# OrientalHorizon/Ray-Tracer-Archive

Measured on NVIDIA B200. Metric: path segments/sec, higher is better.
Workload: dtype f32

## Files before the change

ray_tracer_archive_b200/csrc/rtb_device.cuh:

```cuda
#pragma once
#include <cuda_runtime.h>
#include <stdint.h>

#include <cmath>
#include <cstring>

#include "rtb_internal.hpp"

namespace rtb {

#ifdef RTB_CHECKED
__device__ unsigned int g_rtb_check_fail[8];
enum CheckKind : int { CHK_STACK = 0, CHK_NODE = 1, CHK_PRIM = 2, CHK_SLOT = 3, CHK_QUEUE = 4, CHK_LIST = 5 };
#define RTB_CHECK(kind, cond)                          \
  do {                                                 \
    if (!(cond)) atomicAdd(&g_rtb_check_fail[kind], 1u); \
  } while (0)
#else
#define RTB_CHECK(kind, cond) ((void)0)
#endif

#define RTB_MAX_LIGHTS 8
#define RTB_MAX_MEDIA 8
#define RTB_MAX_CHECKER_DEPTH 8
// ... 70 lines not shown
  uint32_t redo_sel, iter_fixed;
  uint32_t ext_ticket;
  unsigned long long redone;
  unsigned long long refined;
  unsigned long long total_paths;
  unsigned long long segments, rejected;
  unsigned long long nodes_visited, prims_tested;
  unsigned long long prims_tested_type[PT_COUNT];
};

#define RTB_CHUNK 256u
enum SlotClass : uint32_t { CLS_NEW = 6, CLS_DEAD = 7 };
struct DevPool {
  uint32_t n;
  uint32_t n_chunks;
  float4* ray;
  float4* st;
  float4* hit;
  uint8_t* cls;
  uint4* redo[2];
  unsigned long long* cursor;
  DevCounters* c;
};

__device__ __forceinline__ unsigned long long chunk_path(unsigned long long m, uint32_t chunk, uint32_t n_chunks) {
  return (((m >> 5) * n_chunks + chunk) << 5) | (m & 31ull);
}

struct DevParams {
  uint32_t width, height, spp, sample_offset;
  int32_t max_depth;
  uint32_t rr_start, seed;
  float bg[3];
  const uint32_t* pix_order;
  double inv_npix;
  float inv_wm1, inv_hm1;
  uint32_t opt;
  float4* accum;
};

__device__ __forceinline__ float3 f3(float x, float y, float z) { return make_float3(x, y, z); }
__device__ __forceinline__ float3 operator+(float3 a, float3 b) { return f3(a.x + b.x, a.y + b.y, a.z + b.z); }
__device__ __forceinline__ float3 operator-(float3 a, float3 b) { return f3(a.x - b.x, a.y - b.y, a.z - b.z); }
__device__ __forceinline__ float3 operator-(float3 a) { return f3(-a.x, -a.y, -a.z); }
__device__ __forceinline__ float3 operator*(float3 a, float3 b) { return f3(a.x * b.x, a.y * b.y, a.z * b.z); }
__device__ __forceinline__ float3 operator*(float s, float3 a) { return f3(s * a.x, s * a.y, s * a.z); }
__device__ __forceinline__ float3 operator*(float3 a, float s) { return f3(s * a.x, s * a.y, s * a.z); }
__device__ __forceinline__ float dot(float3 a, float3 b) { return fmaf(a.x, b.x, fmaf(a.y, b.y, a.z * b.z)); }
__device__ __forceinline__ float3 cross(float3 a, float3 b) {
  return f3(a.y * b.z - a.z * b.y, a.z * b.x - a.x * b.z, a.x * b.y - a.y * b.x);
}
__device__ __forceinline__ float3 fma3(float s, float3 a, float3 b) {
  return f3(fmaf(s, a.x, b.x), fmaf(s, a.y, b.y), fmaf(s, a.z, b.z));
}
__device__ __forceinline__ float3 unit(float3 a) { return rsqrtf(dot(a, a)) * a; }
__device__ __forceinline__ float3 xyz(float4 a) { return f3(a.x, a.y, a.z); }
__device__ __forceinline__ float3 ld3(const float* p) { return f3(p[0], p[1], p[2]); }

__device__ __forceinline__ float rcp_fast(float x) {
#ifdef __CUDA_ARCH__
  float r;
  asm("rcp.approx.ftz.f32 %0, %1;" : "=f"(r) : "f"(x));
  return r;
#else
  return 1.0f / x;
#endif
}
__device__ __forceinline__ float log_fast(float x) {
#ifdef __CUDA_ARCH__
  return __logf(x);
#else
  return logf(x);
#endif
}
__device__ __forceinline__ float sqrt_fast(float x) {
#ifdef __CUDA_ARCH__
  float r;
  asm("sqrt.approx.ftz.f32 %0, %1;" : "=f"(r) : "f"(x));
  return r;
#else
  return sqrtf(x);
#endif
}

enum RngBlock : uint32_t { BLK_CAMERA0 = 0, BLK_CAMERA1 = 1, BLK_SCATTER = 2, BLK_AUX = 3, BLK_MEDIUM0 = 8 };

__device__ __forceinline__ uint4 philox4(uint32_t pixel, uint32_t sample, uint32_t block, uint32_t bounce, uint32_t seed) {
  uint32_t c0 = block, c1 = bounce, c2 = seed, c3 = 0x52544232u;
  uint32_t k0 = pixel, k1 = sample;
#pragma unroll
  for (int i = 0; i < 10; ++i) {
    uint32_t hi0 = __umulhi(0xD2511F53u, c0), lo0 = 0xD2511F53u * c0;
    uint32_t hi1 = __umulhi(0xCD9E8D57u, c2), lo1 = 0xCD9E8D57u * c2;
    uint32_t n0 = hi1 ^ c1 ^ k0, n2 = hi0 ^ c3 ^ k1;
    c0 = n0; c1 = lo1; c2 = n2; c3 = lo0;
    k0 += 0x9E3779B9u;
    k1 += 0xBB67AE85u;
  }
  return make_uint4(c0, c1, c2, c3);
}
__device__ __forceinline__ float u01(uint32_t x) { return (float)(x >> 8) * (1.0f / 16777216.0f); }
__device__ __forceinline__ float4 philox_u(uint32_t pixel, uint32_t sample, uint32_t block, uint32_t bounce, uint32_t seed) {
  uint4 r = philox4(pixel, sample, block, bounce, seed);
  return make_float4(u01(r.x), u01(r.y), u01(r.z), u01(r.w));
}

struct Closest {
  float t;
  float hi;
  uint32_t ref;
};
#define RTB_U20 9.5367432e-7f
#define RTB_U21 4.7683716e-7f
#define RTB_U22 2.3841858e-7f
#define RTB_U23 1.1920929e-7f
enum HitStatus : int { HIT_MISS = 0, HIT_CERTAIN = 1, HIT_AMBIGUOUS = 2 };
struct TestCount { uint32_t n[PT_COUNT]; };

__device__ __forceinline__ uint32_t ref_gid(const DevScene& sc, uint32_t ref) {
  const uint32_t type = ref >> REF_TYPE_SHIFT, idx = ref & REF_INDEX_MASK;
  return type == PT_MEDIUM ? sc.media[idx].prim_id : __ldg(&sc.info[type][idx].x);
}

__device__ __forceinline__ uint32_t tab_gid(const ExactTab* tab, uint32_t ref) {
  const uint32_t type = ref >> REF_TYPE_SHIFT, idx = ref & REF_INDEX_MASK;
  return type == PT_MEDIUM ? tab->media_prim_id[idx] : __ldg(&tab->info[type][idx].x);
}

__device__ __forceinline__ float abs1(float3 a) { return fabsf(a.x) + fabsf(a.y) + fabsf(a.z); }

#ifdef __CUDA_ARCH__
__device__ __forceinline__ double dadd(double a, double b) { return __dadd_rn(a, b); }
__device__ __forceinline__ double dsub(double a, double b) { return __dsub_rn(a, b); }
__device__ __forceinline__ double dmul(double a, double b) { return __dmul_rn(a, b); }
__device__ __forceinline__ double ddiv(double a, double b) { return __ddiv_rn(a, b); }
__device__ __forceinline__ double dsqrt(double a) { return __dsqrt_rn(a); }
__device__ __forceinline__ uint32_t exact_bits(double v) { return (uint32_t)__double_as_longlong(v); }
#else
__host__ __device__ inline double dadd(double a, double b) { return a + b; }
__host__ __device__ inline double dsub(double a, double b) { return a - b; }
__host__ __device__ inline double dmul(double a, double b) { return a * b; }
__host__ __device__ inline double ddiv(double a, double b) { return a / b; }
__host__ __device__ inline double dsqrt(double a) { return sqrt(a); }
__host__ __device__ inline uint32_t exact_bits(double v) { unsigned long long u; memcpy(&u, &v, 8); return (uint32_t)u; }
#endif
struct D3 { double x, y, z; };
__device__ __forceinline__ D3 d3sub(D3 a, D3 b) { return D3{dsub(a.x, b.x), dsub(a.y, b.y), dsub(a.z, b.z)}; }
__device__ __forceinline__ double d3dot(D3 a, D3 b) {
  return dadd(dadd(dmul(a.x, b.x), dmul(a.y, b.y)), dmul(a.z, b.z));
}
__device__ __forceinline__ D3 d3cross(D3 u, D3 v) {
  return D3{dsub(dmul(u.y, v.z), dmul(u.z, v.y)), -dsub(dmul(u.x, v.z), dmul(u.z, v.x)), dsub(dmul(u.x, v.y), dmul(u.y, v.x))};
}
__device__ __forceinline__ D3 d3at(D3 o, double t, D3 d) {
  return D3{dadd(o.x, dmul(t, d.x)), dadd(o.y, dmul(t, d.y)), dadd(o.z, dmul(t, d.z))};
}

#define RTB_EXACT_MISS (-1.0)
__device__ __forceinline__ double exact_sphere(D3 o, D3 d, D3 c, double r, double tmin) {
  const D3 oc = d3sub(o, c);
  const double a = d3dot(d, d), half_b = d3dot(oc, d);
  const double cc = dsub(d3dot(oc, oc), dmul(r, r));
  const double det = dsub(dmul(half_b, half_b), dmul(a, cc));
  if (det < 0.0) return RTB_EXACT_MISS;
  const double sqrtd = dsqrt(det);
  double root = ddiv(dsub(-half_b, sqrtd), a);
// ... 210 lines not shown
    if (st == HIT_AMBIGUOUS || !(ma > ea && mb > eb)) { t = fmaxf(t - e, 0.0f); return HIT_AMBIGUOUS; }
    return HIT_CERTAIN;
  } else if (type == PT_TRI) {
    const float3 v0 = xyz(__ldg(sc.geom[PT_TRI] + 3 * idx));
    const float3 v1 = xyz(__ldg(sc.geom[PT_TRI] + 3 * idx + 1));
    const float3 v2 = xyz(__ldg(sc.geom[PT_TRI] + 3 * idx + 2));
    const float ax = fabsf(d.x), ay = fabsf(d.y), az = fabsf(d.z);
    const int kz = ax > ay ? (ax > az ? 0 : 2) : (ay > az ? 1 : 2);
    float3 dp = kz == 0 ? f3(d.y, d.z, d.x) : (kz == 1 ? f3(d.z, d.x, d.y) : d);
    float3 A = v0 - o, B = v1 - o, C = v2 - o;
    const float amax = fmaxf(fmaxf(abs1(A), abs1(B)), abs1(C));
    A = kz == 0 ? f3(A.y, A.z, A.x) : (kz == 1 ? f3(A.z, A.x, A.y) : A);
    B = kz == 0 ? f3(B.y, B.z, B.x) : (kz == 1 ? f3(B.z, B.x, B.y) : B);
    C = kz == 0 ? f3(C.y, C.z, C.x) : (kz == 1 ? f3(C.z, C.x, C.y) : C);
    if (dp.z < 0.0f) {
      float s;
      s = dp.x; dp.x = dp.y; dp.y = s;
      s = A.x; A.x = A.y; A.y = s;
      s = B.x; B.x = B.y; B.y = s;
      s = C.x; C.x = C.y; C.y = s;
    }
    const float Sz = rcp_fast(dp.z), Sx = dp.x * Sz, Sy = dp.y * Sz;
    const float Ax = __fsub_rn(A.x, __fmul_rn(Sx, A.z)), Ay = __fsub_rn(A.y, __fmul_rn(Sy, A.z));
    const float Bx = __fsub_rn(B.x, __fmul_rn(Sx, B.z)), By = __fsub_rn(B.y, __fmul_rn(Sy, B.z));
    const float Cx = __fsub_rn(C.x, __fmul_rn(Sx, C.z)), Cy = __fsub_rn(C.y, __fmul_rn(Sy, C.z));
    const float U = __fsub_rn(__fmul_rn(Cx, By), __fmul_rn(Cy, Bx));
    const float V = __fsub_rn(__fmul_rn(Ax, Cy), __fmul_rn(Ay, Cx));
    const float W = __fsub_rn(__fmul_rn(Bx, Ay), __fmul_rn(By, Ax));
    const float m = (1.25f * RTB_U22 * amax) * (fabsf(Ax) + fabsf(Ay) + fabsf(Bx) + fabsf(By) + fabsf(Cx) + fabsf(Cy));
    const float mn = fminf(fminf(U, V), W), mx = fmaxf(fmaxf(U, V), W);
    if (mn < -m && mx > m) return HIT_MISS;
    const float det = U + V + W;
    const float idet = rcp_fast(det), za = Sz * A.z, zb = Sz * B.z, zc = Sz * C.z;
    const float zlo = fminf(fminf(za, zb), zc), zhi = fmaxf(fmaxf(za, zb), zc);
    if (!(mn > m || mx < -m)) {
      if (!(zhi >= tmin)) return HIT_MISS;
      t = fmaxf(zlo - RTB_U20 * fabsf(zlo), 0.0f);
      return HIT_AMBIGUOUS;
    }
    t = (U * za + V * zb + W * zc) * idet;
    e = fmaf(RTB_U20, fabsf(t), 4.0f * m * fabsf(idet) * (zhi - zlo));
    if (!(t - e <= tmax_hi)) return HIT_MISS;
    const int st = tmin_status(t, e, tmin);
    if (st == HIT_AMBIGUOUS) t = fmaxf(t - e, 0.0f);
    return st;
  } else {
    const float4 a = __ldg(sc.geom[PT_MOVING] + 2 * idx);
    const float4 b = __ldg(sc.geom[PT_MOVING] + 2 * idx + 1);
    const float3 c = fma3(time, xyz(b), xyz(a));
    return sphere_fast(o, d, c, a.w, tmin, tmax_hi, t, e, coarse);
  }
}
__device__ __forceinline__ void apply_result(Closest& best, float& amb, uint32_t& flags, int st, float t, float e, uint32_t ref,
                                             bool coarse) {
  if (st == HIT_CERTAIN) consider(best, amb, flags, t, e, ref, coarse);
  else if (st == HIT_AMBIGUOUS) undecided(best, amb, t);
}
template <bool COUNT>
__device__ __forceinline__ void intersect_prim(const DevScene& sc, uint32_t type, uint32_t idx, float3 o, float3 d,
                                               float time, float tmin, Closest& best, float& amb, uint32_t& flags, TestCount& n_tests) {
  float t, e;
  bool coarse;
  const int st = prim_test<COUNT>(sc, type, idx, o, d, time, tmin, best.hi, t, e, coarse, n_tests);
  apply_result(best, amb, flags, st, t, e, (type << REF_TYPE_SHIFT) | idx, coarse);
}

__device__ __forceinline__ float q2f(uint32_t word, uint32_t magic, uint32_t sel) {
  return __uint_as_float(__byte_perm(word, magic, sel));
}

#if !defined(__CUDA_ARCH__) && defined(RTB_EMUL_STATS)
inline unsigned long long g_emul_stats[8];
inline float g_emul_tmax0 = INFINITY;
#endif
struct Trav {
  float3 o, d;
  float idx, idy, idz, time;
  uint32_t octinv;
  uint2 grp;
  int sp;
  Closest best;
  float amb;
};
__device__ __forceinline__ bool needs_exact(const Closest& best, float amb) { return amb < INFINITY && amb <= best.hi; }
enum FixKind : uint32_t { FIX_NONE = 0, FIX_RETRACE = 1, FIX_REFINE = 2 };
#define RTB_REDO_REFINE 0x80000000u
__device__ __forceinline__ bool quad_distance_is_coarse(const DevScene& sc, uint32_t idx, float3 o, float3 d) {
  const float4 w0 = __ldg(sc.geom[PT_QUAD] + 3 * idx);
  if (__ldg(&sc.info[PT_QUAD][idx].y) >> 31) return false;
  const float mag_num = fabsf(w0.w) + fabsf(w0.x * o.x) + fabsf(w0.y * o.y) + fabsf(w0.z * o.z);
  const float mag_den = fabsf(w0.x * d.x) + fabsf(w0.y * d.y) + fabsf(w0.z * d.z);
  return 64.0f * fabsf(dot(xyz(w0), d)) < mag_den || 64.0f * fabsf(w0.w - dot(xyz(w0), o)) < mag_num;
}
__device__ __forceinline__ bool tri_distance_is_coarse(const DevScene& sc, uint32_t idx, float3 o, float3 d) {
  const float3 v0 = xyz(__ldg(sc.geom[PT_TRI] + 3 * idx));
  const float3 n = cross(xyz(__ldg(sc.geom[PT_TRI] + 3 * idx + 1)) - v0, xyz(__ldg(sc.geom[PT_TRI] + 3 * idx + 2)) - v0);
  const float3 r = v0 - o;
  const float mag_num = fabsf(n.x * r.x) + fabsf(n.y * r.y) + fabsf(n.z * r.z);
  const float mag_den = fabsf(n.x * d.x) + fabsf(n.y * d.y) + fabsf(n.z * d.z);
  return 64.0f * fabsf(dot(n, d)) < mag_den || 64.0f * fabsf(dot(n, r)) < mag_num;
}
#define FIX_NOMINATED 3u
__device__ __forceinline__ uint32_t fix_kind_cheap(const Trav& tv) {
  if (needs_exact(tv.best, tv.amb)) return FIX_RETRACE;
  if (tv.best.ref == REF_MISS) return FIX_NONE;
  const uint32_t type = tv.best.ref >> REF_TYPE_SHIFT;
  if (type == PT_QUAD || type == PT_TRI)
    return tv.best.hi - tv.best.t > (type == PT_QUAD ? RTB_FLAT_REL_MAX : RTB_TRI_REL_MAX) * tv.best.t ? FIX_NOMINATED : FIX_NONE;
  return (tv.octinv & RTB_TRAV_COARSE) ? FIX_REFINE : FIX_NONE;
}
__device__ __forceinline__ uint32_t resolve_nominated(const DevScene& sc, uint32_t ref, float3 o, float3 d) {
  const uint32_t type = ref >> REF_TYPE_SHIFT, idx = ref & REF_INDEX_MASK;
  const bool coarse = type == PT_QUAD ? quad_distance_is_coarse(sc, idx, o, d) : tri_distance_is_coarse(sc, idx, o, d);
  return coarse ? FIX_REFINE : FIX_NONE;
}
__device__ __forceinline__ uint32_t fix_kind(const DevScene& sc, const Trav& tv) {
  const uint32_t k = fix_kind_cheap(tv);
  return k == FIX_NOMINATED ? resolve_nominated(sc, tv.best.ref, tv.o, tv.d) : k;
}
__device__ __forceinline__ float slab_lo(const Trav& tv) {
  return tv.best.ref == REF_MISS ? tv.amb : fminf(tv.amb, tv.best.t - (tv.best.hi - tv.best.t));
}

__device__ __forceinline__ void trav_init(Trav& tv, float3 o, float3 d, float time) {
  const float tiny = 1e-30f;
  tv.o = o; tv.d = d; tv.time = time;
  tv.idx = rcp_fast(fabsf(d.x) > tiny ? d.x : copysignf(tiny, d.x));
  tv.idy = rcp_fast(fabsf(d.y) > tiny ? d.y : copysignf(tiny, d.y));
  tv.idz = rcp_fast(fabsf(d.z) > tiny ? d.z : copysignf(tiny, d.z));
  tv.octinv = 7u ^ ((d.x < 0.0f ? 1u : 0u) | (d.y < 0.0f ? 2u : 0u) | (d.z < 0.0f ? 4u : 0u));
  tv.grp = make_uint2(0u, (1u << (tv.octinv + 8)) | 1u);
  tv.sp = 0;
  tv.best = Closest{INFINITY, INFINITY, REF_MISS};
#if !defined(__CUDA_ARCH__) && defined(RTB_EMUL_STATS)
  tv.best.hi = g_emul_tmax0;
#endif
  tv.amb = INFINITY;
}

__device__ __forceinline__ uint4 lds_node_word(const uint4* __restrict__ snodes, uint32_t sbase, uint32_t node, uint32_t w) {
#ifdef __CUDA_ARCH__
  uint4 r;
  asm("ld.shared.v4.u32 {%0, %1, %2, %3}, [%4];" : "=r"(r.x), "=r"(r.y), "=r"(r.z), "=r"(r.w) : "r"(sbase + node * 80u + w * 16u));
  return r;
#else
  return snodes[5 * node + w];
#endif
}

template <class Leaf>
__device__ __forceinline__ void expand_leaves(uint32_t leaf, uint32_t w1y, uint32_t w1z, uint32_t w1w, Leaf&& leaf_fn) {
  const uint32_t ptype = w1y >> REF_TYPE_SHIFT, pbase = w1y & REF_INDEX_MASK;
  uint32_t k = 0;
  while (leaf) {
    const uint32_t s = __ffs(leaf) - 1;
    const uint32_t m = ((s < 4 ? w1z : w1w) >> (8 * (s & 3))) & 0xFFu;
    leaf_fn(ptype, pbase + (m & 31u) + k);
    if (++k >= (m >> 5)) { k = 0; leaf &= leaf - 1; }
  }
}

template <bool COUNT, bool ALL_STAGED, int STRIDE = 1, class Leaves>
__device__ __forceinline__ bool trav_step(const DevScene& sc, const uint4* __restrict__ snodes, uint32_t sbase, uint32_t n_snodes,
                                          Trav& tv, uint2* __restrict__ stack, float tmin,
                                          uint32_t& n_nodes_visited, Leaves&& leaves_fn) {
  if (!(tv.grp.y & 0xFF00u)) {
    if (tv.sp == 0) return false;
    tv.grp = stack[(--tv.sp) * STRIDE];
  }
  const uint32_t octinv = tv.octinv & 7u;
  uint32_t hits = tv.grp.y >> 8;
  const uint32_t prio = 31u - __clz(hits);
  hits &= ~(1u << prio);
  const uint32_t slot = prio ^ octinv;
  const uint32_t gmask = tv.grp.y & 0xFFu;
  const uint32_t node = tv.grp.x + __popc(gmask & ((1u << slot) - 1u));
  RTB_CHECK(CHK_STACK, !hits || tv.sp < RTB_STACK);
  RTB_CHECK(CHK_NODE, node < sc.n_nodes);
  if (hits) stack[(tv.sp++) * STRIDE] = make_uint2(tv.grp.x, (hits << 8) | gmask);
  if (COUNT) ++n_nodes_visited;
  uint4 w0, w1, w2, w3, w4;
  if (ALL_STAGED || node < n_snodes) {
    w0 = lds_node_word(snodes, sbase, node, 0); w1 = lds_node_word(snodes, sbase, node, 1);
    w2 = lds_node_word(snodes, sbase, node, 2); w3 = lds_node_word(snodes, sbase, node, 3);
    w4 = lds_node_word(snodes, sbase, node, 4);
  } else {
    const uint4* p = sc.nodes + 5 * (size_t)node;
    w0 = __ldg(p); w1 = __ldg(p + 1); w2 = __ldg(p + 2); w3 = __ldg(p + 3); w4 = __ldg(p + 4);
  }
  const uint32_t imask = w0.w >> 24;
  const bool nx = !(octinv & 1u), ny = !(octinv & 2u), nz = !(octinv & 4u);
  const float ax = __uint_as_float((w0.w & 0xFFu) << 23) * tv.idx;
  const float ay = __uint_as_float(((w0.w >> 8) & 0xFFu) << 23) * tv.idy;
  const float az = __uint_as_float(((w0.w >> 16) & 0xFFu) << 23) * tv.idz;
  const float bx = (__uint_as_float(w0.x) - tv.o.x) * tv.idx;
  const float by = (__uint_as_float(w0.y) - tv.o.y) * tv.idy;
  const float bz = (__uint_as_float(w0.z) - tv.o.z) * tv.idz;
  const float eps = 5.0e-7f;
  const float ex = eps * fmaf(256.0f, fabsf(ax), fabsf(bx));
  const float ey = eps * fmaf(256.0f, fabsf(ay), fabsf(by));
  const float ez = eps * fmaf(256.0f, fabsf(az), fabsf(bz));
  const float cx = fmaf(-128.0f, ax, bx), cy = fmaf(-128.0f, ay, by), cz = fmaf(-128.0f, az, bz);
  const float bnx = cx - ex, bfx = cx + ex, bny = cy - ey, bfy = cy + ey, bnz = cz - ez, bfz = cz + ez;
  const uint32_t nx0 = nx ? w3.z : w2.x, nx1 = nx ? w3.w : w2.y, fx0 = nx ? w2.x : w3.z, fx1 = nx ? w2.y : w3.w;
  const uint32_t ny0 = ny ? w4.x : w2.z, ny1 = ny ? w4.y : w2.w, fy0 = ny ? w2.z : w4.x, fy1 = ny ? w2.w : w4.y;
  const uint32_t nz0 = nz ? w4.z : w3.x, nz1 = nz ? w4.w : w3.y, fz0 = nz ? w3.x : w4.z, fz1 = nz ? w3.y : w4.w;
  uint32_t missmask = 0;
  const uint32_t magic = sc.prmt_magic;
  const float tmax = tv.best.hi;
#pragma unroll
  for (int i = 7; i >= 0; --i) {
    const uint32_t sel = 0x7044u | ((uint32_t)(i & 3) << 8);
    const float tnx = fmaf(q2f(i < 4 ? nx0 : nx1, magic, sel), ax, bnx);
    const float tny = fmaf(q2f(i < 4 ? ny0 : ny1, magic, sel), ay, bny);
    const float tnz = fmaf(q2f(i < 4 ? nz0 : nz1, magic, sel), az, bnz);
    const float tfx = fmaf(q2f(i < 4 ? fx0 : fx1, magic, sel), ax, bfx);
    const float tfy = fmaf(q2f(i < 4 ? fy0 : fy1, magic, sel), ay, bfy);
    const float tfz = fmaf(q2f(i < 4 ? fz0 : fz1, magic, sel), az, bfz);
    const float tn = fmaxf(fmaxf(tnx, tny), tnz);
    const float tf = fminf(fminf(tfx, tfy), tfz);
    const uint32_t neg = __float_as_uint(tf - tn) | __float_as_uint(tmax - tn) | __float_as_uint(tf - tmin);
    missmask = __funnelshift_l(neg, missmask, 1);
  }
  const uint32_t hitmask = ~missmask & 0xFFu;
#if !defined(__CUDA_ARCH__) && defined(RTB_EMUL_STATS)
  ++g_emul_stats[0];
  if (!hitmask) ++g_emul_stats[1];
  g_emul_stats[2] += __builtin_popcount(hitmask & imask);
  g_emul_stats[3] += __builtin_popcount(hitmask & ~imask);
#endif
  uint32_t ih = hitmask & imask;
  if (octinv & 1u) ih = ((ih & 0x55u) << 1) | ((ih & 0xAAu) >> 1);
  if (octinv & 2u) ih = ((ih & 0x33u) << 2) | ((ih & 0xCCu) >> 2);
  if (octinv & 4u) ih = ((ih & 0x0Fu) << 4) | ((ih & 0xF0u) >> 4);
  tv.grp = make_uint2(w1.x, (ih << 8) | imask);
  const uint32_t leaf = hitmask & ~imask;
  if (leaf) leaves_fn(leaf, w1.y, w1.z, w1.w);
  return true;
}

template <bool COUNT>
__device__ __forceinline__ void trav_globals(const DevScene& sc, Trav& tv, float tmin, TestCount& n_tests) {
  for (uint32_t k = 0; k < sc.n_global; ++k) {
    const uint32_t ref = sc.global_ref[k];
    if ((sc.global_f64 >> k) & 1u) {
      if (COUNT) ++n_tests.n[PT_SPHERE];
      const float4 s = __ldg(sc.geom[PT_SPHERE] + (ref & REF_INDEX_MASK));
      float t;
      const int st = sphere_roots_f64(tv.o, tv.d, xyz(s), s.w, tmin, t);
      if (st == HIT_CERTAIN) consider(tv.best, tv.amb, tv.octinv, t, RTB_U22 * t, ref, false);
      else if (st == HIT_AMBIGUOUS) tv.amb = 0.0f;
    } else {
      intersect_prim<COUNT>(sc, ref >> REF_TYPE_SHIFT, ref & REF_INDEX_MASK, tv.o, tv.d, tv.time, tmin, tv.best, tv.amb, tv.octinv, n_tests);
    }
  }
  if (sc.tree_empty) tv.grp.y = 0u;
}

template <bool COUNT, bool ALL_STAGED = false>
__device__ __forceinline__ bool trav_step_fast(const DevScene& sc, const uint4* __restrict__ snodes, uint32_t sbase, uint32_t n_snodes,
                                               Trav& tv, uint2* __restrict__ stack, float tmin,
                                               uint32_t& n_nodes_visited, TestCount& n_tests) {
  return trav_step<COUNT, ALL_STAGED>(sc, snodes, sbase, n_snodes, tv, stack, tmin, n_nodes_visited,
                                      [&](uint32_t leaf, uint32_t w1y, uint32_t w1z, uint32_t w1w) {
                                        expand_leaves(leaf, w1y, w1z, w1w, [&](uint32_t type, uint32_t idx) {
                                          intersect_prim<COUNT>(sc, type, idx, tv.o, tv.d, tv.time, tmin, tv.best, tv.amb, tv.octinv, n_tests);
                                        });
                                      });
}

template <bool COUNT, bool ALL_STAGED = false>
__device__ __forceinline__ bool trav_step_park(const DevScene& sc, const uint4* __restrict__ snodes, uint32_t sbase, uint32_t n_snodes,
                                               Trav& tv, uint2* __restrict__ stack, float tmin, uint32_t& n_nodes_visited,
                                               uint4* __restrict__ park, bool& parked) {
  return trav_step<COUNT, ALL_STAGED>(sc, snodes, sbase, n_snodes, tv, stack, tmin, n_nodes_visited,
                                      [&](uint32_t leaf, uint32_t w1y, uint32_t w1z, uint32_t w1w) {
                                        *park = make_uint4(leaf, w1y, w1z, w1w);
                                        parked = true;
                                      });
}
template <bool COUNT>
__device__ __forceinline__ void drain_parked(const DevScene& sc, Trav& tv, float tmin, const uint4* __restrict__ park, bool parked,
                                             TestCount& n_tests) {
  uint4 pd = make_uint4(0u, 0u, 0u, 0u);
  if (parked) pd = *park;
  const uint32_t mytype = pd.y >> REF_TYPE_SHIFT;
#pragma unroll
  for (uint32_t t = 0; t < PT_COUNT; ++t) {
    const bool mine = parked && mytype == t;
    if (!__any_sync(0xffffffffu, mine)) continue;
    if (mine)
      expand_leaves(pd.x, pd.y, pd.z, pd.w, [&](uint32_t, uint32_t idx) {
        intersect_prim<COUNT>(sc, t, idx, tv.o, tv.d, tv.time, tmin, tv.best, tv.amb, tv.octinv, n_tests);
      });
    __syncwarp();
  }
}

template <bool COUNT, bool ALL_STAGED = false>
__device__ __forceinline__ uint32_t traverse(const DevScene& sc, const uint4* __restrict__ snodes, uint32_t sbase, uint32_t n_snodes,
                                         float3 o, float3 d, float time, float tmin, Closest& best, float& slab_lo_out,
                                         uint32_t& n_nodes_visited, TestCount& n_tests) {
  Trav tv;
  uint2 stack[RTB_STACK];
  trav_init(tv, o, d, time);
  trav_globals<COUNT>(sc, tv, tmin, n_tests);
  while (trav_step_fast<COUNT, ALL_STAGED>(sc, snodes, sbase, n_snodes, tv, stack, tmin, n_nodes_visited, n_tests)) {}
  best = tv.best;
  slab_lo_out = slab_lo(tv);
  return fix_kind(sc, tv);
}

__device__ __forceinline__ float refine_hit(const DevScene& sc, uint32_t ref, float3 o, float3 d, float time, float t) {
  if ((ref >> REF_TYPE_SHIFT) >= PT_COUNT) return t;
  const double tc = exact_hit(sc.xtab, ref, o, d, time);
  return tc >= 0.0 ? (float)tc : t;
}

__device__ __forceinline__ Closest traverse_exact(const DevScene& sc, float3 o, float3 d, float time, float t_lo = 0.0f, float t_hi = INFINITY) {
  Trav tv;
  uint2 stack[RTB_STACK];
  trav_init(tv, o, d, time);
  tv.best.hi = fmaf(t_hi, 4.0e-6f, t_hi) + 1.0e-6f;
  const float tmin = fmaxf(fmaf(t_lo, -4.0e-6f, t_lo) - 1.0e-6f, 0.0f);
  double bt = 0.0;
  const ExactTab* tab = sc.xtab;
  auto leaf = [&](uint32_t type, uint32_t idx) {
    const uint32_t ref = (type << REF_TYPE_SHIFT) | idx;
    {
      Closest probe{INFINITY, tv.best.hi, REF_MISS};
      float probe_amb = INFINITY;
      uint32_t probe_flags = 0;
      TestCount none{};
      intersect_prim<false>(sc, type, idx, tv.o, tv.d, tv.time, RTB_TMIN, probe, probe_amb, probe_flags, none);
      if (probe.ref == REF_MISS && !(probe_amb < INFINITY)) return;
    }
    const double tc = exact_hit(tab, ref, tv.o, tv.d, tv.time);
    if (tc < 0.0) return;
    if (tv.best.ref == REF_MISS || tc < bt || (tc == bt && tab_gid(tab, ref) > tab_gid(tab, tv.best.ref))) {
      bt = tc;
      const float tf = (float)tc;
      tv.best.t = tf;
      tv.best.hi = tf * (1.0f + RTB_U22);
      tv.best.ref = ref;
    }
  };
  for (uint32_t k = 0; k < sc.n_global; ++k) leaf(sc.global_ref[k] >> REF_TYPE_SHIFT, sc.global_ref[k] & REF_INDEX_MASK);
  if (sc.tree_empty) tv.grp.y = 0u;
  uint32_t nv = 0;
  while (trav_step<false, false>(sc, nullptr, 0u, 0u, tv, stack, tmin, nv,
                                 [&](uint32_t lf, uint32_t w1y, uint32_t w1z, uint32_t w1w) { expand_leaves(lf, w1y, w1z, w1w, leaf); })) {}
  if (tv.best.ref == REF_MISS) tv.best.t = tv.best.hi = INFINITY;
  return tv.best;
}

__device__ __forceinline__ void intersect_media(const DevScene& sc, float3 o, float3 d, float tmin, Closest& best,
                                                uint32_t pixel, uint32_t sample, uint32_t bounce, uint32_t seed,
                                                bool have_rng) {
  for (uint32_t m = 0; m < sc.n_media; ++m) {
    const DevMedium& md = sc.media[m];
    float t1, t2;
    if (md.boundary_type == RTB_BOUNDARY_SPHERE) {
      float3 c = f3(md.p[0], md.p[1], md.p[2]);
      float3 oc = o - c;
      float a = dot(d, d), hb = dot(oc, d), inv_a = rcp_fast(a);
      float3 l = fma3(-hb * inv_a, d, oc);
      float disc = fmaf(md.p[3], md.p[3], -dot(l, l));
      if (disc < 0.0f) continue;
      float sq = sqrt_fast(a * disc);
      t1 = (-hb - sq) * inv_a;
      t2 = (-hb + sq) * inv_a;
      if (t2 < t1 + 0.0001f) continue;
    } else {
      float3 oo = o - f3(md.off[0], md.off[1], md.off[2]);
      float3 ro = f3(md.cos_t * oo.x - md.sin_t * oo.z, oo.y, md.sin_t * oo.x + md.cos_t * oo.z);
      float3 rd = f3(md.cos_t * d.x - md.sin_t * d.z, d.y, md.sin_t * d.x + md.cos_t * d.z);
      float lo = -INFINITY, hi = INFINITY;
      const float ro_[3] = {ro.x, ro.y, ro.z}, rd_[3] = {rd.x, rd.y, rd.z};
      bool miss = false;
#pragma unroll
      for (int a = 0; a < 3; ++a) {
        if (rd_[a] == 0.0f) {
          if (ro_[a] < md.p[a] || ro_[a] > md.p[3 + a]) miss = true;
          continue;
        }
        float inv = rcp_fast(rd_[a]);
        float ta = (md.p[a] - ro_[a]) * inv, tb = (md.p[3 + a] - ro_[a]) * inv;
        lo = fmaxf(lo, fminf(ta, tb));
        hi = fminf(hi, fmaxf(ta, tb));
      }
// ... 21 lines not shown
```

ray_tracer_archive_b200/csrc/rtb_kernels.cu:

```cuda
#include <cuda_runtime.h>

#include <algorithm>
#include <cstdlib>
#include <cstring>

#include "rtb_device.cuh"
#include "rtb_launch.hpp"

namespace rtb {

__device__ __forceinline__ uint32_t ray_octant(float3 d) {
  return (d.x < 0.0f ? 1u : 0u) | (d.y < 0.0f ? 2u : 0u) | (d.z < 0.0f ? 4u : 0u);
}

__device__ __forceinline__ void prefetch_l1(const void* p) { asm volatile("prefetch.global.L1 [%0];" ::"l"(p)); }
__device__ __forceinline__ void prefetch_l2(const void* p) { asm volatile("prefetch.global.L2 [%0];" ::"l"(p)); }

__device__ __forceinline__ void red_add_v4(float4* addr, float a, float b, float c, float d) {
  asm volatile("red.global.add.v4.f32 [%0], {%1, %2, %3, %4};" ::"l"(addr), "f"(a), "f"(b), "f"(c), "f"(d) : "memory");
}

__device__ __forceinline__ void deposit(const DevParams& prm, DevCounters* c, uint32_t pixel, float3 L) {
  if (!(isfinite(L.x) && isfinite(L.y) && isfinite(L.z))) {
    atomicAdd(&c->rejected, 1ull);
    return;
  }
  const float Y = 0.2126f * L.x + 0.7152f * L.y + 0.0722f * L.z;
  red_add_v4(prm.accum + pixel, L.x, L.y, L.z, Y * Y);
}

__device__ __forceinline__ void prefetch_chunk_rays(const DevPool& pool, uint32_t chunk_base, uint32_t lane) {
  const char* rp = reinterpret_cast<const char*>(pool.ray + 2 * (size_t)chunk_base);
  prefetch_l2(rp + 128u * lane);
  prefetch_l2(rp + 128u * (lane + 32u));
}

__device__ __forceinline__ void stage_nodes(const DevScene& sc, uint4* snodes, uint32_t n_snodes) {
  const uint32_t words = n_snodes * 5u;
  for (uint32_t i = threadIdx.x; i < words; i += blockDim.x) snodes[i] = __ldg(sc.nodes + i);
  __syncthreads();
}

__device__ __forceinline__ void finish_ray(const DevScene& sc, const DevPool& pool, const DevParams& prm, uint32_t slot,
                                           float3 o, float3 d, Closest best) {
  if (sc.n_media) {
    const uint32_t pixel = __float_as_uint(pool.st[2 * slot].w);
    const uint32_t st = __float_as_uint(pool.st[2 * slot + 1].w);
    intersect_media(sc, o, d, RTB_TMIN, best, pixel, st >> 8, (st & 0xFFu) + 1u, prm.seed, !(prm.opt & RTB_OPT_PROBE));
  }
  uint32_t queue = Q_TERMINAL, minfo = 0;
  if (best.ref != REF_MISS) {
    const uint32_t type = best.ref >> REF_TYPE_SHIFT, idx = best.ref & REF_INDEX_MASK;
    minfo = type == PT_MEDIUM ? sc.media[idx].minfo : __ldg(&sc.info[type][idx].y);
    queue = RTB_MINFO_QUEUE(minfo);
  }
  RTB_CHECK(CHK_SLOT, slot < pool.n);
  pool.hit[slot] = make_float4(best.t, __uint_as_float(best.ref), __uint_as_float(minfo), 0.f);
  pool.cls[slot] = (uint8_t)queue;
}

__device__ __forceinline__ void queue_fix(const DevPool& pool, uint32_t slot, uint32_t kind, float lo, float hi) {
  const uint32_t qi = atomicAdd(&pool.c->redo_count[0], 1u);
  RTB_CHECK(CHK_QUEUE, qi < pool.n && slot < pool.n);
  pool.redo[0][qi] =
      make_uint4(slot | (kind == FIX_REFINE ? RTB_REDO_REFINE : 0u), __float_as_uint(lo), __float_as_uint(hi), 0u);
}

__device__ __forceinline__ void finish_ray(const DevScene& sc, const DevPool& pool, const DevParams& prm, uint32_t slot,
                                           float3 o, float3 d, Closest best);
static __device__ __noinline__ uint32_t fix_one(const DevScene* __restrict__ dsc, float4* ray, float4* st, float4* hit, uint8_t* cls,
                                                DevCounters* c, uint4 q, uint32_t seed, uint32_t opt) {
  const DevScene& sc = *dsc;
  DevPool pool;
  pool.n = 0xFFFFFFFFu; pool.n_chunks = 0;
  pool.ray = ray; pool.st = st; pool.hit = hit; pool.cls = cls;
  pool.redo[0] = pool.redo[1] = nullptr; pool.cursor = nullptr; pool.c = c;
  DevParams prm;
  prm.seed = seed; prm.opt = opt;
  const uint32_t slot = q.x & ~RTB_REDO_REFINE;
  const float4 ro = ray[2 * slot], rd = ray[2 * slot + 1];
  if (q.x & RTB_REDO_REFINE) {
    const float4 h = hit[slot];
    hit[slot].x = refine_hit(sc, __float_as_uint(h.y), xyz(ro), xyz(rd), ro.w, h.x);
    return 1u;
  }
  const Closest best = traverse_exact(sc, xyz(ro), xyz(rd), ro.w, __uint_as_float(q.y), __uint_as_float(q.z));
  finish_ray(sc, pool, prm, slot, xyz(ro), xyz(rd), best);
  return 0u;
}

__device__ __forceinline__ uint2 fix_prologue(const DevScene& sc, const DevPool& pool, const DevParams& prm, uint32_t warp_in_grid,
                                              uint32_t n_warps_in_grid, uint32_t lane) {
  const uint32_t n = pool.c->redo_count[0];
  uint2 done = make_uint2(0u, 0u);
  for (uint32_t i = warp_in_grid * 32u + lane; i < n; i += n_warps_in_grid * 32u) {
    done.y += fix_one(sc.self, pool.ray, pool.st, pool.hit, pool.cls, pool.c, pool.redo[0][i], prm.seed, prm.opt);
    ++done.x;
  }
  return done;
}

__device__ __forceinline__ uint32_t append_class(uint2 cw, uint32_t key, uint8_t* list, uint32_t len, uint32_t lane) {
  const uint32_t e0 = __vcmpeq4(cw.x & 0x07070707u, key * 0x01010101u), e1 = __vcmpeq4(cw.y & 0x07070707u, key * 0x01010101u);
  const uint32_t cnt = (__popc(e0) + __popc(e1)) >> 3;
  uint32_t incl = cnt;
#pragma unroll
  for (uint32_t d = 1; d < 32; d <<= 1) {
    const uint32_t v = __shfl_up_sync(0xffffffffu, incl, d);
    if (lane >= d) incl += v;
  }
  const uint32_t total = __shfl_sync(0xffffffffu, incl, 31);
  if (total) {
    uint32_t pos = len + incl - cnt;
#pragma unroll
    for (uint32_t j = 0; j < 8; ++j)
      if (((j < 4 ? e0 : e1) >> (8 * (j & 3))) & 1u) {
        RTB_CHECK(CHK_LIST, pos < RTB_CHUNK);
        list[pos++] = (uint8_t)(8u * lane + j);
      }
  }
  return len + total;
}

// ... 348 lines not shown
      rdy_lo |= __reduce_or_sync(0xffffffffu, !again && r < 32u ? 1u << r : 0u);
      rdy_hi |= __reduce_or_sync(0xffffffffu, !again && (r & 32u) ? 1u << (r & 31u) : 0u);
      __syncwarp();
      if (again) W.q[cls][(head + q_max + __popc(again_mask & lt_mask)) & 63u] = (uint8_t)r;
      const uint32_t delta = __popc(again_mask) - n;
      if (cls == 0u) { qh0 += n; qn0 += delta; } else if (cls == 1u) { qh1 += n; qn1 += delta; } else { qh2 += n; qn2 += delta; }
      __syncwarp();
      continue;
    }
    if ((rdy_lo >> lane) & 1u) W.ready[__popc(rdy_lo & lt_mask)] = (uint8_t)lane;
    if ((rdy_hi >> lane) & 1u) W.ready[__popc(rdy_lo) + __popc(rdy_hi & lt_mask)] = (uint8_t)(32u + lane);
    __syncwarp();
    flip ^= 1u;
    bool finished = false, leafed = false;
    uint32_t cls = 3u, r = 64u;
    if (lane < n_ready) {
      r = W.ready[lane + (flip && n_ready > 32u ? n_ready - 32u : 0u)];
      Trav tv;
      const float4 ro = W.o_time[r], id = W.idir_oct[r];
      const uint4 tr = W.trav[r];
      tv.o = xyz(ro);
      tv.idx = id.x; tv.idy = id.y; tv.idz = id.z;
      tv.octinv = __float_as_uint(id.w);
      tv.grp = make_uint2(tr.x, tr.y);
      tv.sp = (int)tr.z;
      tv.best.hi = W.best[r].z;
      finished = !trav_step<COUNT, false, (int)RTB_WQ_RAYS>(sc, snodes, sbase, n_snodes, tv, &W.stack[0][r], RTB_TMIN, nv,
                                                            [&](uint32_t leaf, uint32_t w1y, uint32_t w1z, uint32_t w1w) {
                                                              W.rec[r] = make_uint4(leaf, w1y, w1z, w1w);
                                                              const uint32_t type = w1y >> REF_TYPE_SHIFT;
                                                              cls = type <= PT_MOVING ? 0u : type - 1u;
                                                              leafed = true;
                                                            });
      RTB_CHECK(CHK_STACK, tv.sp <= (int)RTB_WQ_STACK);
      if (!finished) {
        *reinterpret_cast<uint2*>(&W.trav[r]) = tv.grp;
        W.trav[r].z = (uint32_t)tv.sp;
      }
    }
    const uint32_t done = __ballot_sync(0xffffffffu, finished);
    const uint32_t leafs = __ballot_sync(0xffffffffu, leafed);
    if (done | leafs) {
      const uint32_t bit_lo = r < 32u ? 1u << r : 0u, bit_hi = (r & 32u) ? 1u << (r & 31u) : 0u;
      rdy_lo &= ~__reduce_or_sync(0xffffffffu, finished || leafed ? bit_lo : 0u);
      rdy_hi &= ~__reduce_or_sync(0xffffffffu, finished || leafed ? bit_hi : 0u);
      if (leafs) {
        const uint32_t m0 = __ballot_sync(0xffffffffu, cls == 0u), m1 = __ballot_sync(0xffffffffu, cls == 1u), m2 = leafs & ~(m0 | m1);
        if (leafed) {
          const uint32_t mine = cls == 0u ? m0 : (cls == 1u ? m1 : m2);
          const uint32_t end = cls == 0u ? qh0 + qn0 : (cls == 1u ? qh1 + qn1 : qh2 + qn2);
          W.q[cls][(end + __popc(mine & lt_mask)) & 63u] = (uint8_t)r;
        }
        qn0 += __popc(m0); qn1 += __popc(m1); qn2 += __popc(m2);
      }
      if (done) {
        free_lo |= __reduce_or_sync(0xffffffffu, finished ? bit_lo : 0u);
        free_hi |= __reduce_or_sync(0xffffffffu, finished ? bit_hi : 0u);
        if (out_count + __popc(done) > 32u) flush();
        if (finished) {
          const float4 b = W.best[r];
          Trav tv;
          tv.best = Closest{b.x, b.z, __float_as_uint(b.y)};
          tv.amb = b.w;
          tv.octinv = W.trav[r].w;
          W.out[out_count + __popc(done & lt_mask)] =
              ExtOut{tv.best.t, tv.best.ref, __float_as_uint(W.d_slot[r].w), fix_kind_cheap(tv), slab_lo(tv), tv.best.hi, {0u, 0u}};
        }
        out_count += __popc(done);
      }
    }
    __syncwarp();
  }
  if (lane == 0 && n_rays) atomicAdd(&c->iter_rays, n_rays);
  if (COUNT) report_counts(c, nv, nt, lane);
}

template <bool COUNT, bool ALL_STAGED, bool SORT>
__global__ void __maxnreg__(RTB_EXTEND_MAXREG)
k_extend_static(DevScene sc, DevPool pool, DevParams prm, uint32_t n_snodes) {
  extern __shared__ uint4 snodes[];
  __shared__ uint8_t s_list[RTB_EXTEND_WARPS][RTB_CHUNK];
  __shared__ uint32_t s_cnt[SORT ? RTB_EXTEND_WARPS : 1][64];
  DevCounters* c = pool.c;
  stage_nodes(sc, snodes, n_snodes);
  uint32_t sbase = (uint32_t)__cvta_generic_to_shared(snodes);
  asm volatile("mov.u32 %0, %0;" : "+r"(sbase));
  const uint32_t lane = threadIdx.x & 31u, warp = threadIdx.x >> 5;
  uint8_t* list = s_list[warp];
  const uint32_t n_warps = gridDim.x * RTB_EXTEND_WARPS;
  uint32_t n_rays = 0, nv = 0;
  TestCount nt{};
  for (uint32_t chunk = blockIdx.x * RTB_EXTEND_WARPS + warp; chunk < pool.n_chunks; chunk += n_warps) {
    const uint32_t base = chunk * RTB_CHUNK;
    const uint32_t total = SORT ? build_extend_list_sorted(pool, chunk, list, s_cnt[SORT ? warp : 0], lane) : build_extend_list(pool, chunk, list, lane);
    n_rays += total;
    for (uint32_t r = 0; r < total; r += 32) {
      if (r + 32 + lane < total) prefetch_l1(pool.ray + 2 * (size_t)(base + list[r + 32 + lane]));
      if (r + lane < total) {
        const uint32_t slot = base + list[r + lane];
        const float4 ro = pool.ray[2 * slot];
        const float4 rd = pool.ray[2 * slot + 1];
        Closest best;
        float lo;
        const uint32_t fix = traverse<COUNT, ALL_STAGED>(sc, snodes, sbase, n_snodes, xyz(ro), xyz(rd), ro.w, RTB_TMIN, best, lo, nv, nt);
        finish_ray(sc, pool, prm, slot, xyz(ro), xyz(rd), best);
        if (fix) queue_fix(pool, slot, fix, lo, best.hi);
      }
    }
    __syncwarp();
  }
  if (lane == 0 && n_rays) atomicAdd(&c->iter_rays, n_rays);
  if (COUNT) report_counts(c, nv, nt, lane);
}

struct Surf {
  float3 p, n, outward;
  bool front;
  uint32_t mat, ref;
};

__device__ __forceinline__ Surf surface_at(const DevScene& sc, uint32_t ref, uint32_t minfo, float3 o, float3 d, float time, float t) {
  Surf s;
  s.ref = ref;
  s.p = fma3(t, d, o);
  const uint32_t type = ref >> REF_TYPE_SHIFT, idx = ref & REF_INDEX_MASK;
  if (type == PT_MEDIUM) {
    s.n = s.outward = f3(1.f, 0.f, 0.f);
    s.front = true;
    s.mat = RTB_MINFO_MAT(minfo);
    return s;
  }
  if (type == PT_SPHERE) {
    const float4 g = __ldg(sc.geom[PT_SPHERE] + idx);
    s.outward = rcp_fast(g.w) * (s.p - xyz(g));
  } else if (type == PT_MOVING) {
    const float4 a = __ldg(sc.geom[PT_MOVING] + 2 * idx), b = __ldg(sc.geom[PT_MOVING] + 2 * idx + 1);
    s.outward = rcp_fast(a.w) * (s.p - fma3(time, xyz(b), xyz(a)));
  } else if (type == PT_QUAD) {
    s.outward = xyz(__ldg(sc.geom[PT_QUAD] + 3 * idx));
  } else {
    const float3 v0 = xyz(__ldg(sc.geom[PT_TRI] + 3 * idx));
    const float3 e1 = xyz(__ldg(sc.geom[PT_TRI] + 3 * idx + 1)) - v0, e2 = xyz(__ldg(sc.geom[PT_TRI] + 3 * idx + 2)) - v0;
    s.outward = unit(cross(e1, e2));
  }
  s.mat = RTB_MINFO_MAT(minfo);
  bool ff = dot(d, s.outward) < 0.0f;
  s.n = ff ? s.outward : -s.outward;
  const uint32_t mode = RTB_MINFO_FACE(minfo), base = mode & 7u;
  if (mode >= FACE_Q) {
    float sn, cs;
    if (type == PT_TRI) {
      sn = __ldg(sc.geom[PT_TRI] + 3 * idx).w;
      cs = __ldg(sc.geom[PT_TRI] + 3 * idx + 1).w;
    } else {
      const double* ex = sc.xtab->exact[type] + (size_t)idx * RTB_EXACT_STRIDE;
      sn = (float)ex[4]; cs = (float)ex[5];
    }
    const bool q = dot(f3(cs * d.x - sn * d.z, d.y, sn * d.x + cs * d.z), s.n) < 0.0f;
    s.front = base == FACE_Q ? q : base == FACE_NOT_Q ? !q : base == FACE_NATURAL ? ff : base == FACE_FLIPPED ? !ff : base == FACE_TRUE;
    if ((mode & FACE_BARE) && !q) s.n = -s.n;
  } else {
    s.front = base == FACE_NATURAL ? ff : base == FACE_FLIPPED ? !ff : base == FACE_TRUE;
  }
  return s;
}

__device__ __forceinline__ void surface_uv(const DevScene& sc, const Surf& s, float& u, float& v) {
  const uint32_t type = s.ref >> REF_TYPE_SHIFT, idx = s.ref & REF_INDEX_MASK;
  u = v = 0.f;
  if (type == PT_SPHERE) {
    const double* ex = sc.xtab->exact[PT_SPHERE] + (size_t)idx * RTB_EXACT_STRIDE;
    const float sn = (float)ex[4], cs = (float)ex[5];
    const float3 on = f3(cs * s.outward.x - sn * s.outward.z, s.outward.y, sn * s.outward.x + cs * s.outward.z);
    const float theta = acosf(fminf(fmaxf(-on.y, -1.f), 1.f));
    const float phi = atan2f(-on.z, on.x) + RTB_PI;
    u = phi / (2.0f * RTB_PI);
    v = theta / RTB_PI;
  } else if (type == PT_QUAD) {
    const float4 w1 = __ldg(sc.geom[PT_QUAD] + 3 * idx + 1), w2 = __ldg(sc.geom[PT_QUAD] + 3 * idx + 2);
    u = dot(xyz(w1), s.p) - w1.w;
    v = dot(xyz(w2), s.p) - w2.w;
  } else if (type == PT_TRI) {
    const float3 v0 = xyz(__ldg(sc.geom[PT_TRI] + 3 * idx)), e1 = xyz(__ldg(sc.geom[PT_TRI] + 3 * idx + 1)) - v0,
                 e2 = xyz(__ldg(sc.geom[PT_TRI] + 3 * idx + 2)) - v0;
    const float3 nn = cross(e1, e2), pl = s.p - v0;
    const float inv = 1.0f / dot(nn, nn);
    u = dot(nn, cross(pl, e2)) * inv;
// ... 728 lines not shown
```

Measured before the change: 7701.

## Use packed f32x2 slab math and shared octant lookup table in BVH traversal

Adds Blackwell packed f32x2 FMA/sub helpers and rewrites the 8-child slab test to process two children per packed instruction. It also replaces the three conditional bit-swizzles that reorder the child hit mask by octant with a 2 KB shared-memory lookup table filled at kernel start. Both paths are enabled only in the static extend kernel when all nodes are staged in shared memory (packed math only when not counting). The goal is fewer ALU instructions per node visit, at the cost of extra pack/unpack moves, a shared-memory load per node, and a little more shared memory per block.

```diff
diff --git a/ray_tracer_archive_b200/csrc/rtb_device.cuh b/ray_tracer_archive_b200/csrc/rtb_device.cuh
--- a/ray_tracer_archive_b200/csrc/rtb_device.cuh
+++ b/ray_tracer_archive_b200/csrc/rtb_device.cuh
@@ -176,6 +176,45 @@
   return sqrtf(x);
 #endif
 }
+
+#ifdef __CUDA_ARCH__
+__device__ __forceinline__ unsigned long long pk2(float2 a) {
+  unsigned long long r;
+  asm("mov.b64 %0, {%1, %2};" : "=l"(r) : "f"(a.x), "f"(a.y));
+  return r;
+}
+__device__ __forceinline__ float2 upk2(unsigned long long r) {
+  float2 a;
+  asm("mov.b64 {%0, %1}, %2;" : "=f"(a.x), "=f"(a.y) : "l"(r));
+  return a;
+}
+__device__ __forceinline__ float2 ffma2(float2 a, float2 b, float2 c) {
+  unsigned long long r;
+  asm("fma.rn.f32x2 %0, %1, %2, %3;" : "=l"(r) : "l"(pk2(a)), "l"(pk2(b)), "l"(pk2(c)));
+  return upk2(r);
+}
+__device__ __forceinline__ float2 fadd2(float2 a, float2 b) {
+  unsigned long long r;
+  asm("add.rn.f32x2 %0, %1, %2;" : "=l"(r) : "l"(pk2(a)), "l"(pk2(b)));
+  return upk2(r);
+}
+__device__ __forceinline__ float2 fsub2(float2 a, float2 b) {
+  unsigned long long r;
+  asm("sub.rn.f32x2 %0, %1, %2;" : "=l"(r) : "l"(pk2(a)), "l"(pk2(b)));
+  return upk2(r);
+}
+__device__ __forceinline__ float2 fmul2(float2 a, float2 b) {
+  unsigned long long r;
+  asm("mul.rn.f32x2 %0, %1, %2;" : "=l"(r) : "l"(pk2(a)), "l"(pk2(b)));
+  return upk2(r);
+}
+#else
+__device__ __forceinline__ float2 ffma2(float2 a, float2 b, float2 c) { return make_float2(fmaf(a.x, b.x, c.x), fmaf(a.y, b.y, c.y)); }
+__device__ __forceinline__ float2 fadd2(float2 a, float2 b) { return make_float2(a.x + b.x, a.y + b.y); }
+__device__ __forceinline__ float2 fsub2(float2 a, float2 b) { return make_float2(a.x - b.x, a.y - b.y); }
+__device__ __forceinline__ float2 fmul2(float2 a, float2 b) { return make_float2(a.x * b.x, a.y * b.y); }
+#endif
+__device__ __forceinline__ float2 f2s(float s) { return make_float2(s, s); }
 
 enum RngBlock : uint32_t { BLK_CAMERA0 = 0, BLK_CAMERA1 = 1, BLK_SCATTER = 2, BLK_AUX = 3, BLK_MEDIUM0 = 8 };
 
@@ -552,6 +591,13 @@
   Closest best;
   float amb;
 };
+__device__ __forceinline__ uint32_t octant_remap(uint32_t m, uint32_t octinv) {
+  if (octinv & 1u) m = ((m & 0x55u) << 1) | ((m & 0xAAu) >> 1);
+  if (octinv & 2u) m = ((m & 0x33u) << 2) | ((m & 0xCCu) >> 2);
+  if (octinv & 4u) m = ((m & 0x0Fu) << 4) | ((m & 0xF0u) >> 4);
+  return m;
+}
+__shared__ uint8_t s_octmap[8 * 256];
 __device__ __forceinline__ bool needs_exact(const Closest& best, float amb) { return amb < INFINITY && amb <= best.hi; }
 enum FixKind : uint32_t { FIX_NONE = 0, FIX_RETRACE = 1, FIX_REFINE = 2 };
 #define RTB_REDO_REFINE 0x80000000u
@@ -630,7 +676,7 @@
   }
 }
 
-template <bool COUNT, bool ALL_STAGED, int STRIDE = 1, class Leaves>
+template <bool COUNT, bool ALL_STAGED, int STRIDE = 1, bool PACKED = false, bool OCTMAP = false, class Leaves>
 __device__ __forceinline__ bool trav_step(const DevScene& sc, const uint4* __restrict__ snodes, uint32_t sbase, uint32_t n_snodes,
                                           Trav& tv, uint2* __restrict__ stack, float tmin,
                                           uint32_t& n_nodes_visited, Leaves&& leaves_fn) {
@@ -675,22 +721,43 @@
   const uint32_t nx0 = nx ? w3.z : w2.x, nx1 = nx ? w3.w : w2.y, fx0 = nx ? w2.x : w3.z, fx1 = nx ? w2.y : w3.w;
   const uint32_t ny0 = ny ? w4.x : w2.z, ny1 = ny ? w4.y : w2.w, fy0 = ny ? w2.z : w4.x, fy1 = ny ? w2.w : w4.y;
   const uint32_t nz0 = nz ? w4.z : w3.x, nz1 = nz ? w4.w : w3.y, fz0 = nz ? w3.x : w4.z, fz1 = nz ? w3.y : w4.w;
-  uint32_t missmask = 0;
   const uint32_t magic = sc.prmt_magic;
   const float tmax = tv.best.hi;
+  uint32_t missmask;
+  if constexpr (PACKED) {
+    uint32_t mlo = 0, mhi = 0;
 #pragma unroll
-  for (int i = 7; i >= 0; --i) {
-    const uint32_t sel = 0x7044u | ((uint32_t)(i & 3) << 8);
-    const float tnx = fmaf(q2f(i < 4 ? nx0 : nx1, magic, sel), ax, bnx);
-    const float tny = fmaf(q2f(i < 4 ? ny0 : ny1, magic, sel), ay, bny);
-    const float tnz = fmaf(q2f(i < 4 ? nz0 : nz1, magic, sel), az, bnz);
-    const float tfx = fmaf(q2f(i < 4 ? fx0 : fx1, magic, sel), ax, bfx);
-    const float tfy = fmaf(q2f(i < 4 ? fy0 : fy1, magic, sel), ay, bfy);
-    const float tfz = fmaf(q2f(i < 4 ? fz0 : fz1, magic, sel), az, bfz);
-    const float tn = fmaxf(fmaxf(tnx, tny), tnz);
-    const float tf = fminf(fminf(tfx, tfy), tfz);
-    const uint32_t neg = __float_as_uint(tf - tn) | __float_as_uint(tmax - tn) | __float_as_uint(tf - tmin);
-    missmask = __funnelshift_l(neg, missmask, 1);
+    for (int i = 3; i >= 0; --i) {
+      const uint32_t sel = 0x7044u | ((uint32_t)i << 8);
+      const float2 tnx = ffma2(make_float2(q2f(nx0, magic, sel), q2f(nx1, magic, sel)), f2s(ax), f2s(bnx));
+      const float2 tny = ffma2(make_float2(q2f(ny0, magic, sel), q2f(ny1, magic, sel)), f2s(ay), f2s(bny));
+      const float2 tnz = ffma2(make_float2(q2f(nz0, magic, sel), q2f(nz1, magic, sel)), f2s(az), f2s(bnz));
+      const float2 tfx = ffma2(make_float2(q2f(fx0, magic, sel), q2f(fx1, magic, sel)), f2s(ax), f2s(bfx));
+      const float2 tfy = ffma2(make_float2(q2f(fy0, magic, sel), q2f(fy1, magic, sel)), f2s(ay), f2s(bfy));
+      const float2 tfz = ffma2(make_float2(q2f(fz0, magic, sel), q2f(fz1, magic, sel)), f2s(az), f2s(bfz));
+      const float2 tn = make_float2(fmaxf(fmaxf(tnx.x, tny.x), tnz.x), fmaxf(fmaxf(tnx.y, tny.y), tnz.y));
+      const float2 tf = make_float2(fminf(fminf(tfx.x, tfy.x), tfz.x), fminf(fminf(tfx.y, tfy.y), tfz.y));
+      const float2 d = fsub2(tf, tn);
+      mlo = __funnelshift_l(__float_as_uint(d.x) | __float_as_uint(tmax - tn.x) | __float_as_uint(tf.x - tmin), mlo, 1);
+      mhi = __funnelshift_l(__float_as_uint(d.y) | __float_as_uint(tmax - tn.y) | __float_as_uint(tf.y - tmin), mhi, 1);
+    }
+    missmask = (mhi << 4) | mlo;
+  } else {
+    missmask = 0;
+#pragma unroll
+    for (int i = 7; i >= 0; --i) {
+      const uint32_t sel = 0x7044u | ((uint32_t)(i & 3) << 8);
+      const float tnx = fmaf(q2f(i < 4 ? nx0 : nx1, magic, sel), ax, bnx);
+      const float tny = fmaf(q2f(i < 4 ? ny0 : ny1, magic, sel), ay, bny);
+      const float tnz = fmaf(q2f(i < 4 ? nz0 : nz1, magic, sel), az, bnz);
+      const float tfx = fmaf(q2f(i < 4 ? fx0 : fx1, magic, sel), ax, bfx);
+      const float tfy = fmaf(q2f(i < 4 ? fy0 : fy1, magic, sel), ay, bfy);
+      const float tfz = fmaf(q2f(i < 4 ? fz0 : fz1, magic, sel), az, bfz);
+      const float tn = fmaxf(fmaxf(tnx, tny), tnz);
+      const float tf = fminf(fminf(tfx, tfy), tfz);
+      const uint32_t neg = __float_as_uint(tf - tn) | __float_as_uint(tmax - tn) | __float_as_uint(tf - tmin);
+      missmask = __funnelshift_l(neg, missmask, 1);
+    }
   }
   const uint32_t hitmask = ~missmask & 0xFFu;
 #if !defined(__CUDA_ARCH__) && defined(RTB_EMUL_STATS)
@@ -700,9 +767,8 @@
   g_emul_stats[3] += __builtin_popcount(hitmask & ~imask);
 #endif
   uint32_t ih = hitmask & imask;
-  if (octinv & 1u) ih = ((ih & 0x55u) << 1) | ((ih & 0xAAu) >> 1);
-  if (octinv & 2u) ih = ((ih & 0x33u) << 2) | ((ih & 0xCCu) >> 2);
-  if (octinv & 4u) ih = ((ih & 0x0Fu) << 4) | ((ih & 0xF0u) >> 4);
+  if constexpr (OCTMAP) ih = s_octmap[(octinv << 8) | ih];
+  else ih = octant_remap(ih, octinv);
   tv.grp = make_uint2(w1.x, (ih << 8) | imask);
   const uint32_t leaf = hitmask & ~imask;
   if (leaf) leaves_fn(leaf, w1.y, w1.z, w1.w);
@@ -727,11 +793,11 @@
   if (sc.tree_empty) tv.grp.y = 0u;
 }
 
-template <bool COUNT, bool ALL_STAGED = false>
+template <bool COUNT, bool ALL_STAGED = false, bool PACKED = false, bool OCTMAP = false>
 __device__ __forceinline__ bool trav_step_fast(const DevScene& sc, const uint4* __restrict__ snodes, uint32_t sbase, uint32_t n_snodes,
                                                Trav& tv, uint2* __restrict__ stack, float tmin,
                                                uint32_t& n_nodes_visited, TestCount& n_tests) {
-  return trav_step<COUNT, ALL_STAGED>(sc, snodes, sbase, n_snodes, tv, stack, tmin, n_nodes_visited,
+  return trav_step<COUNT, ALL_STAGED, 1, PACKED, OCTMAP>(sc, snodes, sbase, n_snodes, tv, stack, tmin, n_nodes_visited,
                                       [&](uint32_t leaf, uint32_t w1y, uint32_t w1z, uint32_t w1w) {
                                         expand_leaves(leaf, w1y, w1z, w1w, [&](uint32_t type, uint32_t idx) {
                                           intersect_prim<COUNT>(sc, type, idx, tv.o, tv.d, tv.time, tmin, tv.best, tv.amb, tv.octinv, n_tests);
@@ -743,7 +809,7 @@
 __device__ __forceinline__ bool trav_step_park(const DevScene& sc, const uint4* __restrict__ snodes, uint32_t sbase, uint32_t n_snodes,
                                                Trav& tv, uint2* __restrict__ stack, float tmin, uint32_t& n_nodes_visited,
                                                uint4* __restrict__ park, bool& parked) {
-  return trav_step<COUNT, ALL_STAGED>(sc, snodes, sbase, n_snodes, tv, stack, tmin, n_nodes_visited,
+  return trav_step<COUNT, ALL_STAGED, 1, false>(sc, snodes, sbase, n_snodes, tv, stack, tmin, n_nodes_visited,
                                       [&](uint32_t leaf, uint32_t w1y, uint32_t w1z, uint32_t w1w) {
                                         *park = make_uint4(leaf, w1y, w1z, w1w);
                                         parked = true;
@@ -767,7 +833,7 @@
   }
 }
 
-template <bool COUNT, bool ALL_STAGED = false>
+template <bool COUNT, bool ALL_STAGED = false, bool PACKED = false, bool OCTMAP = false>
 __device__ __forceinline__ uint32_t traverse(const DevScene& sc, const uint4* __restrict__ snodes, uint32_t sbase, uint32_t n_snodes,
                                          float3 o, float3 d, float time, float tmin, Closest& best, float& slab_lo_out,
                                          uint32_t& n_nodes_visited, TestCount& n_tests) {
@@ -775,7 +841,7 @@
   uint2 stack[RTB_STACK];
   trav_init(tv, o, d, time);
   trav_globals<COUNT>(sc, tv, tmin, n_tests);
-  while (trav_step_fast<COUNT, ALL_STAGED>(sc, snodes, sbase, n_snodes, tv, stack, tmin, n_nodes_visited, n_tests)) {}
+  while (trav_step_fast<COUNT, ALL_STAGED, PACKED, OCTMAP>(sc, snodes, sbase, n_snodes, tv, stack, tmin, n_nodes_visited, n_tests)) {}
   best = tv.best;
   slab_lo_out = slab_lo(tv);
   return fix_kind(sc, tv);
diff --git a/ray_tracer_archive_b200/csrc/rtb_kernels.cu b/ray_tracer_archive_b200/csrc/rtb_kernels.cu
--- a/ray_tracer_archive_b200/csrc/rtb_kernels.cu
+++ b/ray_tracer_archive_b200/csrc/rtb_kernels.cu
@@ -39,6 +39,10 @@
   const uint32_t words = n_snodes * 5u;
   for (uint32_t i = threadIdx.x; i < words; i += blockDim.x) snodes[i] = __ldg(sc.nodes + i);
   __syncthreads();
+}
+
+__device__ __forceinline__ void octmap_fill() {
+  for (uint32_t i = threadIdx.x; i < 8u * 256u; i += blockDim.x) s_octmap[i] = (uint8_t)octant_remap(i & 0xFFu, i >> 8);
 }
 
 __device__ __forceinline__ void finish_ray(const DevScene& sc, const DevPool& pool, const DevParams& prm, uint32_t slot,
@@ -553,6 +557,7 @@
   __shared__ uint8_t s_list[RTB_EXTEND_WARPS][RTB_CHUNK];
   __shared__ uint32_t s_cnt[SORT ? RTB_EXTEND_WARPS : 1][64];
   DevCounters* c = pool.c;
+  if constexpr (ALL_STAGED) octmap_fill();
   stage_nodes(sc, snodes, n_snodes);
   uint32_t sbase = (uint32_t)__cvta_generic_to_shared(snodes);
   asm volatile("mov.u32 %0, %0;" : "+r"(sbase));
@@ -573,7 +578,7 @@
         const float4 rd = pool.ray[2 * slot + 1];
         Closest best;
         float lo;
-        const uint32_t fix = traverse<COUNT, ALL_STAGED>(sc, snodes, sbase, n_snodes, xyz(ro), xyz(rd), ro.w, RTB_TMIN, best, lo, nv, nt);
+        const uint32_t fix = traverse<COUNT, ALL_STAGED, ALL_STAGED && !COUNT, ALL_STAGED>(sc, snodes, sbase, n_snodes, xyz(ro), xyz(rd), ro.w, RTB_TMIN, best, lo, nv, nt);
         finish_ray(sc, pool, prm, slot, xyz(ro), xyz(rd), best);
         if (fix) queue_fix(pool, slot, fix, lo, best.hi);
       }
```

Result: faster. 8002, median of 6 (+3.9%).
